# whatshap/whatshap

Hardware: AMD Instinct MI355X
Metric: variant-columns/sec at max-coverage 20 (bipartition-costs/sec reported alongside) (higher is better)
Workload: dtype u32; 1 GPU; synthetic diploid single-individual, max-coverage 20: 1 block of 200000 SNVs (BASELINE configs[2]); blocks=1, blocks_in_flight_per_gpu=1, tables_per_launch=1, max_coverage=20, optimal_cost_checksum=1611545, rendezvous=none

## Files before the change

### whatshap_amd/csrc/dp_device.hip

```cpp
#include <hip/hip_runtime.h>

#include <algorithm>
#include <atomic>
#include <cctype>
#include <chrono>
#include <cstdio>
#include <cstdlib>
#include <cstring>
#include <mutex>
#include <string>
#include <vector>

#include "debug_build.h"
#include "device_pool.h"
#include "device_table.h"
#include "genotype.h"

namespace whamd {

#define HIP_TRY(expr)                                                                                 \
	do {                                                                                              \
		hipError_t err_ = (expr);                                                                     \
		if (err_ != hipSuccess) {                                                                     \
			msg = std::string(#expr) + " failed: " + hipGetErrorString(err_);                         \
// ... 516 lines not shown
		schedule.clear();
		entries.clear();
		slot_entries.clear();
		windows.clear();
	}

	void release() {
		if (tail_elsewhere && ev3) (void)hipEventSynchronize(ev3);
		tail_elsewhere = false;
		if (upload_pending && ev_upload) (void)hipEventSynchronize(ev_upload);
		upload_pending = false;
		release_lanes();
		windowed = false;
		if (stream && own_stream_used && (!allocations.empty() || d_arena)) { (void)hipStreamSynchronize(stream); own_stream_used = false; }
		for (auto& a : allocations) devpool_give(device, a.first, a.second);
		allocations.clear();
		arena_give(device, d_arena, arena_bytes);
		d_arena = nullptr;
		arena_bytes = 0;
		pinned_give(h_pinned, h_pinned_bytes);
		h_pinned = nullptr;
		d_cols = nullptr;
		d_units = nullptr;
		d_pr[0] = d_pr[1] = nullptr;
		d_path_index = d_path_trans = d_score = nullptr;
	}
};

DeviceTable::DeviceTable() : impl_(new Impl()) {}

DeviceTable::~DeviceTable() {
	if (impl_) {
		release_device();
		delete impl_;
	}
}

void DeviceTable::release_device() {
	Impl& m = *impl_;
	(void)hipSetDevice(m.device);
	m.release();
	if (m.stream) {
		if (m.own_stream_used) (void)hipStreamSynchronize(m.stream);
		m.own_stream_used = false;
		StreamSet ss;
		ss.stream = m.stream; ss.ev[0] = m.ev0; ss.ev[1] = m.ev1; ss.ev[2] = m.ev2; ss.ev[3] = m.ev3; ss.ev[4] = m.ev_group; ss.ev[5] = m.ev_upload; ss.device = m.device;
		streamset_give(ss);
	}
	m.stream = m.run_stream = nullptr;
	m.ev0 = m.ev1 = m.ev2 = m.ev3 = m.ev_group = m.ev_upload = nullptr;
	m.timing_pending = false;
}

int DeviceTable::device_count() {
	int n = 0;
	if (hipGetDeviceCount(&n) != hipSuccess) return 0;
	return n;
}

bool DeviceTable::device_pci_bus_id(int device, std::string& out) {
	int n = 0;
	if (hipGetDeviceCount(&n) != hipSuccess || device < 0 || device >= n) return false;
	char text[64] = {0};
	if (hipDeviceGetPCIBusId(text, (int)sizeof text - 1, device) != hipSuccess) return false;
	out = text;
	for (char& ch : out) ch = (char)tolower((unsigned char)ch);
	return true;
}

static void append_segments(uint32_t mask, std::vector<uint32_t>& out, uint16_t& count) {
	uint32_t src = 0;
	count = 0;
	for (uint32_t bit = 0; bit < 32;) {
		if (!((mask >> bit) & 1u)) { ++bit; continue; }
		uint32_t len = 0;
		while (bit + len < 32 && ((mask >> (bit + len)) & 1u)) ++len;
		out.push_back(src | (bit << 8) | (len << 16));
		++count;
		src += len;
		bit += len;
	}
}

bool DeviceTable::set_path(const std::string& path) {
	if (path != "auto" && path != "column" && path != "column_keys" && path != "resident" && path != "slots") return false;
	impl_->path = path;
	return true;
}

void DeviceTable::set_l_pref(int l) { impl_->l_pref = std::max(4, std::min(l, RES_LMAX)); }
void DeviceTable::set_lanes(int n) { impl_->max_lanes = n < 1 ? 1 : (n > 64 ? 64 : n); }

void DeviceTable::set_fold(bool v) { impl_->fold = v; }
void DeviceTable::set_slot_l(int l) { impl_->slot_l = std::max(2, std::min(l, 12)); impl_->slot_l_set = true; }
void DeviceTable::set_slot_lr(int lr) { impl_->slot_lr = lr >= 3 ? 3 : (lr <= 1 ? 1 : 2); }

void DeviceTable::set_arena_limit(uint64_t bytes) { impl_->arena_limit = bytes; }
void DeviceTable::set_shared_launches(bool v) { impl_->shared_hint = v; }
void DeviceTable::set_side_by_side(bool v) { impl_->side_by_side = v; }
void DeviceTable::set_symmetry(int level) { impl_->symmetry = level < 0 ? 0 : (level > 2 ? 2 : level); }

whamd_status_t DeviceTable::upload(Problem& p, int device, std::string& msg) {
	Impl& m = *impl_;
	m.device = device;
	int ndev = 0;
	if (hipGetDeviceCount(&ndev) != hipSuccess || ndev <= 0) {
		msg = "no HIP device visible: the whatshap_amd device path needs an MI355X (gfx950); there is no CPU fallback";
		return WHAMD_ERR_DEVICE;
	}
	if (device < 0 || device >= ndev) {
		msg = "device index " + std::to_string(device) + " out of range (" + std::to_string(ndev) + " visible)";
		return WHAMD_ERR_DEVICE;
	}
	HIP_TRY(hipSetDevice(device));
	if (!m.stream) {
		StreamSet ss;
		if (!streamset_take(device, ss)) { msg = "could not create the table's stream and events"; return WHAMD_ERR_DEVICE; }
		m.stream = ss.stream; m.ev0 = ss.ev[0]; m.ev1 = ss.ev[1]; m.ev2 = ss.ev[2]; m.ev3 = ss.ev[3]; m.ev_group = ss.ev[4]; m.ev_upload = ss.ev[5];
	}
	m.release();
	const uint32_t n = p.n_cols;
	if (n == 0) return WHAMD_OK;
	m.wide = !select_kernels(p.T, p.n_ind, m.fused, m.keysfn);
	if (m.wide && (p.T > (uint32_t)MAX_T_WIDE || p.n_ind > (uint32_t)MAX_IND_WIDE)) {
		msg = "no device kernel for T=" + std::to_string(p.T) + ", individuals=" + std::to_string(p.n_ind);
		return WHAMD_ERR_UNSUPPORTED;
	}
	for (uint32_t c = 0; c < p.n_cols && !m.wide; ++c) m.wide = p.term_end(c, p.T - 1) - p.term_begin(c, 0) > (uint64_t)COL_MAXTERMS;
	const bool force_keys = m.path == "column_keys" || m.wide;
	const bool want_resident = (m.path == "auto" || m.path == "resident") && !m.wide;
	const auto tu0 = std::chrono::steady_clock::now();
	size_t free_b = 0, total_b = 0;
	HIP_TRY(hipMemGetInfo(&free_b, &total_b));
	if (free_b < total_b / 2) {
		genotype_release_cache();
		HIP_TRY(hipMemGetInfo(&free_b, &total_b));
	}
	if (free_b < total_b / 4) {
		dptable_release_arena_cache();
		devpool_release();
		HIP_TRY(hipMemGetInfo(&free_b, &total_b));
	}
	free_b += arena_idle_bytes(device);
	int slot_lr = m.slot_lr, slot_l = m.slot_l;
	if (m.shared_hint && p.T == 1 && p.max_k >= 18 && !m.slot_l_set && m.slot_lr == 2) { slot_lr = 3; slot_l = 12; }
	if (p.T == 1 && p.max_k >= 21 && p.max_k <= 22 && !m.slot_l_set && m.slot_lr == 2 && !debug_env("WHAMD_NO_WIDE_LAYOUT")) { slot_lr = 3; slot_l = 12; }
	m.slot_lr_used = slot_lr;
	m.use_slots = (m.path == "auto" || m.path == "slots") && !m.wide && plan_forward_slots(p, p.T > 1 ? (m.slot_l_set ? -m.slot_l : 0) : std::max(8, slot_l), m.symmetry, m.splan, slot_lr);
	if (m.use_slots && m.splan.ped && m.splan.table_words * 4ull > free_b / 4) m.use_slots = false;
	m.table_bytes = m.use_slots && m.splan.ped ? m.splan.table_words * 4ull : 0ull;
	if (p.lazy_terms) {
		std::vector<uint8_t> need(p.n_cols, 1);
		if (m.use_slots && m.splan.ped) for (uint32_t c = 0; c < p.n_cols; ++c) need[c] = m.splan.col_to_row[c] < 0;
		const whamd_status_t st = fill_lazy_terms(p, need, msg);
		if (st != WHAMD_OK) return st;
	}
	if (m.use_slots) {
		m.plan = ResidentPlan();
		m.plan.steps = m.splan.steps;
		m.plan.component_first_step = m.splan.component_first_step;
		m.plan.col_to_res.assign(p.n_cols, -1);
	} else {
		m.splan = SlotPlan();
		plan_forward(p, want_resident, m.l_pref, m.fold, m.plan, m.symmetry);
	}
	const auto tu1 = std::chrono::steady_clock::now();
	if (debug_env("WHAMD_DEBUG_PLAN")) {
		for (const Step& st : m.plan.steps) {
			if (st.kind == 0) { fprintf(stderr, "[plan] column %u k=%u b=%u f=%u\n", st.index, p.k[st.index], p.b[st.index], p.f[st.index]); continue; }
			if (st.kind == 2) {
				const SlotRun& r = m.splan.runs[st.index];
				fprintf(stderr, "[plan] slot run c0=%u ncols=%u g=%u L=%u half=%u ends=%u has_prev=%u in_identity=%u in_half=%u mirror_pos=%u in_occ=%x out_occ=%x mirror_out=%u\n",
				        r.c0, r.ncols, r.g, r.L, r.half, r.n_ends, r.has_prev, r.in_identity, r.in_half, r.in_mirror_pos, r.in_occ, r.out_occ, r.mirror_out);
				if (m.splan.ped) fprintf(stderr, "[plan]   pedigree run: T=%u forms per value=%u table words=%u record words per workgroup=%u\n", 1u << m.splan.pextra[st.index].tb,
				                         m.splan.pextra[st.index].nf, m.splan.pextra[st.index].s_off + r.ncols * 64u * pslot_ns(m.splan.pextra[st.index].nf), m.splan.pextra[st.index].rec_words);
				continue;
			}
			const ResSegment& sgm = m.plan.segments[st.index];
			fprintf(stderr, "[plan] run c0=%u ncols=%u g=%u threads=%u max_l=%u stage_words=%u\n", sgm.c0, sgm.ncols, sgm.g, sgm.threads, sgm.max_l, sgm.stage_words);
			for (uint32_t i = 0; i < sgm.ncols; ++i) {
				const ResColumn& rc = m.plan.columns[sgm.col_off + i];
				const ResBacktrace& rb = m.plan.backtrace[sgm.col_off + i];
				fprintf(stderr, "[plan]   col %u mode=%u nfold=%u Lb=%u Lf=%u ebits=%u epos0=%u nthr=%u stage_off=%u nwords=%u | bt layout=%u n_g=%u n_l=%u\n",
				        sgm.c0 + i, rc.mode, rc.nfold, rc.Lb, rc.Lf, rc.ebits, rc.epos[0], rc.nthr, rc.stage_off, rc.nwords, rb.layout, rb.n_g, rb.n_l);
			}
		}
	}
	const uint32_t tbits = 2 * p.n_triples;
	const uint32_t ni = std::max<uint32_t>(p.n_ind, 1);
	const bool timing = getenv("WHAMD_DEBUG_TIMING") != nullptr;
	auto lap_t = std::chrono::steady_clock::now();
	auto ulap = [&](const char* what) {
		if (!timing) return;
		const auto now = std::chrono::steady_clock::now();
		fprintf(stderr, "[whamd timing]   upload: %s %.2f ms\n", what, std::chrono::duration<double, std::milli>(now - lap_t).count());
		lap_t = now;
	};
	m.cols.resize(n);
	std::vector<uint32_t> segs;
	RawVec<uint32_t> term_ptr32((size_t)n * (p.T + 1));
	static_assert(sizeof(CostTerm) == sizeof(DevTerm), "Problem::terms / fterms are uploaded as they are");
	const RawVec<CostTerm>& terms = p.terms;
	if (p.terms.size() >= 0xFFFFFFFFull || (uint64_t)p.col_ptr[n] * ni >= 0xFFFFFFFFull) {
		msg = "problem too large for 32-bit device offsets";
		return WHAMD_ERR_UNSUPPORTED;
	}
	uint64_t bt = 0, seg_bt = 0;
	size_t seg_cursor = 0, slot_cursor = 0;
	uint32_t max_f = 0, max_keys_f = 0;
	const uint64_t reserve = (3ull << 30) + (uint64_t)n * 1024ull + m.table_bytes;
	const bool ped_slots = m.use_slots && m.splan.ped;
	auto slot_record_bytes = [&](size_t ri) -> uint64_t {
		const SlotRun& run = m.splan.runs[ri];
		if (ped_slots) return (uint64_t)m.splan.pextra[ri].rec_words * 4ull << run.g;
		return (uint64_t)run.n_ends * run.threads * (1ull << (run.g - run.half));
	};
	uint64_t arena_cap = free_b > reserve ? free_b - reserve : 0;
	if (m.arena_limit) arena_cap = std::min<uint64_t>(arena_cap, m.arena_limit);
	std::vector<uint32_t> window_first_col;
	uint64_t bt_max = 0;
	auto open_unit = [&](uint32_t c, uint64_t bytes) -> bool {
		if (bytes + 16 > arena_cap) return false;
		if (bt + bytes + 16 > arena_cap) {
			bt_max = std::max(bt_max, bt);
			bt = 0;
			window_first_col.push_back(c);
		}
		return true;
	};
	auto unit_too_large = [&](uint32_t c) {
		msg = "the backtrace record of the unit at column " + std::to_string(c) + " alone does not fit in the arena (" + std::to_string(arena_cap >> 20) +
		      " MiB of " + std::to_string(free_b >> 20) + " MiB free HBM)";
		return WHAMD_ERR_UNSUPPORTED;
	};
	parallel_ranges(n, host_threads(n, 16384), [&](uint64_t c0, uint64_t c1, uint32_t) {
		for (uint32_t c = (uint32_t)c0; c < (uint32_t)c1; ++c) {
			DevColumn d{};
			d.k = p.k[c];
			d.b = p.b[c];
			d.f = p.f[c];
			d.recomb = p.recomb[c];
			d.delta_off = (uint32_t)(p.col_ptr[c] * ni);
			d.term_off = (uint32_t)((size_t)c * (p.T + 1));
			for (uint32_t t = 0; t <= p.T; ++t) term_ptr32[(size_t)c * (p.T + 1) + t] = (uint32_t)p.term_ptr[(size_t)c * p.T + t];
			d.ebits = d.k - d.f;
			d.is_last = (c + 1 == n);
			d.eloop = std::min<uint32_t>(d.ebits, QMAX);
			d.nplanes = d.ebits + tbits;
			m.cols[c] = d;
		}
	});
	for (uint32_t c = 0; c < n; ++c) {
		DevColumn& d = m.cols[c];
		const bool in_slot_run = m.use_slots && m.splan.col_to_row[c] >= 0;
		d.seg_off = (uint32_t)segs.size();
		const uint32_t kmask = d.k >= 32 ? 0xFFFFFFFFu : ((1u << d.k) - 1u);
		if (!in_slot_run) {
			append_segments(p.fwd_mask[c], segs, d.nseg_fwd);
			append_segments(kmask & ~p.fwd_mask[c], segs, d.nseg_end);
		}
		d.bt_off = bt;
		if (m.use_slots && m.splan.col_to_row[c] >= 0) {
			d.mode = 3;
			d.res_idx = (uint32_t)m.splan.col_to_row[c];
			if (slot_cursor < m.splan.runs.size() && m.splan.runs[slot_cursor].c0 == c) {
				SlotRun& run = m.splan.runs[slot_cursor];
				if (!open_unit(c, slot_record_bytes(slot_cursor))) return unit_too_large(c);
				run.rec_lo = (uint32_t)bt;
				run.rec_hi = (uint32_t)(bt >> 32);
				seg_bt = bt;
				bt += slot_record_bytes(slot_cursor);
				max_f = std::max(max_f, run.L + run.g);
				++slot_cursor;
			}
			d.bt_off = seg_bt;
		} else if (m.plan.col_to_res[c] >= 0) {
			d.mode = 2;
			d.res_idx = (uint32_t)m.plan.col_to_res[c];
			if (seg_cursor < m.plan.segments.size() && m.plan.segments[seg_cursor].c0 == c) {
				ResSegment& sgm = m.plan.segments[seg_cursor];
				if (!open_unit(c, (uint64_t)sgm.stage_words * (1ull << sgm.g) * 8ull)) return unit_too_large(c);
				sgm.bt_lo = (uint32_t)bt;
				sgm.bt_hi = (uint32_t)(bt >> 32);
				seg_bt = bt;
				bt += (uint64_t)sgm.stage_words * (1ull << sgm.g) * 8ull;
				++seg_cursor;
			}
			d.bt_off = seg_bt;
		} else {
			const bool fused_ok = !force_keys && !d.is_last && d.f >= 6 && d.ebits <= (uint32_t)QMAX;
			d.mode = fused_ok ? 0u : 1u;
			const uint64_t bytes = d.mode == 0 ? (uint64_t)d.nplanes * p.T * (1ull << (d.f - 6)) * 8ull : (uint64_t)p.T * (1ull << d.f) * 4ull;
			if (!open_unit(c, bytes)) return unit_too_large(c);
			d.bt_off = bt;
			bt += bytes;
			if (d.mode != 0) max_keys_f = std::max(max_keys_f, d.f);
		}
		bt = (bt + 15ull) & ~15ull;
		max_f = std::max(max_f, d.f);
	}
	ulap("column descriptors (host)");
	bt = bt_max = std::max(bt_max, bt);
	m.bt_bytes = bt;
	m.windowed = !window_first_col.empty();
	m.checkpoint_bytes = (size_t)(1ull << max_f) * p.T * 4;
	const uint64_t need = bt + (2ull + window_first_col.size()) * (1ull << max_f) * p.T * 4ull + (1ull << max_keys_f) * p.T * 8ull;
	if (need + (1ull << 30) > free_b) {
		msg = "backtrace arena of " + std::to_string(need >> 20) + " MiB does not fit in free HBM (" + std::to_string(free_b >> 20) + " MiB)";
		return WHAMD_ERR_UNSUPPORTED;
	}
	hipStream_t us = debug_env("WHAMD_UPLOAD_ON_TABLE_STREAM") ? nullptr : upload_stream_of(device);
	if (!us) us = m.stream;
	m.upload_stream = us;
	if (us == m.stream) m.own_stream_used = true;
	StageSession stage(us);
	ulap("staging area taken");
	auto alloc = [&](void** dptr, size_t bytes) -> hipError_t {
		size_t got = 0;
		hipError_t e = devpool_take(device, std::max<size_t>(bytes, 16), dptr, &got);
		if (e == hipSuccess) m.allocations.emplace_back(*dptr, got);
		return e;
	};
	std::vector<int32_t> delta_fallback;
	const int32_t* delta_src = p.delta.data();
	size_t delta_count = (size_t)p.col_ptr[n] * p.n_ind;
	if (p.n_ind == 0) { delta_fallback.assign(std::max<size_t>(p.col_ptr[n], 1), 0); delta_src = delta_fallback.data(); delta_count = delta_fallback.size(); }
	void *d_delta, *d_term_ptr, *d_terms, *d_segs, *d_bt, *d_keys, *d_last_keys, *d_rcol, *d_rbt, *d_fterms = nullptr;
	m.device_superreads = n > 0 && p.n_ind == 1 && p.T == 1 && p.P == 2 && !p.distrust && p.h2p.size() >= 2 && p.h2p[0] == 0 && p.h2p[1] == 1 && p.genotype.size() >= n &&
	                      !debug_env("WHAMD_HOST_SUPERREADS");
	const size_t super_upload = m.device_superreads ? ((size_t)n + 1) * 8 + n + 1024 : 0;
	const size_t upload_bytes = m.cols.size() * sizeof(DevColumn) + delta_count * sizeof(int32_t) + term_ptr32.size() * 4 + (terms.size() + p.fterms.size()) * sizeof(DevTerm) + segs.size() * 4 +
	             m.plan.columns.size() * (sizeof(ResColumn) + sizeof(ResBacktrace) + sizeof(PedColumn)) + m.plan.ped_terms.size() * sizeof(PedTerm) +
	             (m.splan.rows.size() + SLOT_ROW_PAD) * sizeof(SlotRow) + m.splan.prows.size() * sizeof(PedSlotRow) + m.splan.bt_cols.size() * (sizeof(SlotBtCol) + 8) +
	             m.splan.runs.size() * (sizeof(SlotRun) + sizeof(PedSlotExtra) + sizeof(BtUnit) + sizeof(SlotBatchEntry) + 64) + m.plan.segments.size() * (sizeof(ResBatchEntry) + sizeof(BtUnit)) + super_upload + ((size_t)8 << 20);
	stage.expect(upload_bytes);
// ... 103 lines not shown
		m.super_words = (size_t)n + ((size_t)2 * n + 3) / 4;
	}
	if (!p.fterms.empty()) HIP_TRY(up(&d_fterms, p.fterms.data(), p.fterms.size() * sizeof(DevTerm)));
	HIP_TRY(up(&d_segs, segs.data(), segs.size() * sizeof(uint32_t)));
	HIP_TRY(up(&d_rcol, m.plan.columns.data(), m.plan.columns.size() * sizeof(ResColumn)));
	HIP_TRY(up(&d_rbt, m.plan.backtrace.data(), m.plan.backtrace.size() * sizeof(ResBacktrace)));
	void *d_pcol = nullptr, *d_pterm = nullptr;
	m.plan.ped_columns.resize(m.plan.ped_columns.empty() ? 0 : m.plan.columns.size());
	HIP_TRY(up(&d_pcol, m.plan.ped_columns.data(), m.plan.ped_columns.size() * sizeof(PedColumn)));
	HIP_TRY(up(&d_pterm, m.plan.ped_terms.data(), m.plan.ped_terms.size() * sizeof(PedTerm)));
	m.dp.ped_cols = (const PedColumn*)d_pcol;
	m.dp.ped_terms = (const PedTerm*)d_pterm;
	ulap("column arrays: allocations + copies");
	RawVec<uint32_t> slot_blob;
	std::vector<uint32_t> slot_blob_off(m.splan.runs.size(), 0), slot_blob_words(m.splan.runs.size(), 0);
	{
		size_t words = 0;
		for (size_t ri = 0; ri < m.splan.runs.size(); ++ri) {
			const SlotRun& run = m.splan.runs[ri];
			slot_blob_off[ri] = (uint32_t)words;
			slot_blob_words[ri] = (uint32_t)((size_t)run.ncols * (sizeof(SlotBtCol) / 4) + (run.n_ends + 3) / 4 + 1);
			words += slot_blob_words[ri];
		}
		slot_blob.resize(words);
		parallel_ranges(m.splan.runs.size(), host_threads(m.splan.runs.size(), 512), [&](uint64_t r0, uint64_t r1, uint32_t) {
			for (size_t ri = r0; ri < r1; ++ri) {
				const SlotRun& run = m.splan.runs[ri];
				uint32_t* dst = slot_blob.data() + slot_blob_off[ri];
				const size_t col_words = (size_t)run.ncols * (sizeof(SlotBtCol) / 4);
				std::memcpy(dst, m.splan.bt_cols.data() + run.row_off, col_words * 4);
				const size_t end_words = (run.n_ends + 3) / 4 + 1;
				std::memset(dst + col_words, 0, end_words * 4);
				if (run.n_ends) std::memcpy(dst + col_words, m.splan.end_slots.data() + m.splan.end_off[ri], run.n_ends);
			}
		});
	}
	ulap("slot backtrace blobs (host)");
	void *d_srows = nullptr, *d_sblob = nullptr;
	if (!m.splan.rows.empty()) m.splan.rows.resize(m.splan.rows.size() + SLOT_ROW_PAD);
	HIP_TRY(up(&d_srows, m.splan.rows.data(), m.splan.rows.size() * sizeof(SlotRow)));
	ulap("slot rows: allocation + copy");
	HIP_TRY(up(&d_sblob, slot_blob.data(), slot_blob.size() * sizeof(uint32_t)));
	void* d_sctrl = nullptr;
	HIP_TRY(up(&d_sctrl, m.splan.ctrl.data(), m.splan.ctrl.size() * sizeof(uint32_t)));
	m.dp.slot_ctrl = (const uint32_t*)d_sctrl;
	void *d_sruns = nullptr, *d_stab = nullptr;
	uint64_t slot_tab_words = 0;
	if (m.use_slots && !ped_slots) {
		for (SlotRun& run : m.splan.runs) {
			auto pad4 = [](uint64_t v) { return (v + 3ull) & ~3ull; };
			const bool xrun = (run.yflags & 1u) && (run.lr == 2u || (run.lr == 3u && !debug_env("WHAMD_NO_XRUN8"))) && run.ncols <= (uint32_t)SLOT_XCOLS &&
			                  run.n_ends <= (uint32_t)SLOT_XENDS && !debug_env("WHAMD_NO_XRUN");
			const uint64_t ncp = xrun ? ((run.ncols + 7u) & ~7u) : run.ncols;
			run.tab_g = (uint32_t)slot_tab_words;
			slot_tab_words += pad4(ncp << (run.g - run.half));
			run.tab_w = (uint32_t)slot_tab_words;
			slot_tab_words += pad4(ncp * (run.threads >> 6));
			run.tab_sl = (uint32_t)slot_tab_words;
			slot_tab_words += ncp * 64u;
			if (xrun) {
				run.yflags |= 8u;
				slot_tab_words = (slot_tab_words + 15u) & ~(uint64_t)15;
				run.tab_kr = (uint32_t)slot_tab_words;
				slot_tab_words += pad4((((uint64_t)run.ncols + SLOT_XPAD) << run.lr) + run.ncols + SLOT_XPAD);
				run.tab_par = (uint32_t)slot_tab_words;
				slot_tab_words += pad4((uint64_t)run.threads + (1ull << (run.g - run.half)));
			}
		}
		slot_tab_words += (uint64_t)SLOT_XCOLS * 64u;
		if (getenv("WHAMD_DEBUG_TIMING")) {
			size_t nx = 0, not_y = 0, not_lr = 0, long_run = 0, many_ends = 0;
			for (const SlotRun& run : m.splan.runs) {
				nx += (run.yflags & 8u) != 0;
				not_y += !(run.yflags & 1u); not_lr += run.lr != 2u && run.lr != 3u; long_run += run.ncols > (uint32_t)SLOT_XCOLS; many_ends += run.n_ends > (uint32_t)SLOT_XENDS;
			}
			fprintf(stderr, "[whamd timing]   X runs: %zu of %zu (not Y form %zu, cells per thread %zu, more than %d columns %zu, more than %d ending reads %zu)\n", nx, m.splan.runs.size(), not_y,
			        not_lr, SLOT_XCOLS, long_run, SLOT_XENDS, many_ends);
		}
		if (slot_tab_words >= 0xFFFFFFFFull) { msg = "slot-run tables exceed 32-bit offsets"; return WHAMD_ERR_UNSUPPORTED; }
		HIP_TRY(up(&d_sruns, m.splan.runs.data(), m.splan.runs.size() * sizeof(SlotRun)));
		ulap("slot blobs, control words, runs: allocations + copies");
		HIP_TRY(alloc(&d_stab, slot_tab_words * 4));
		ulap("slot tables: allocation");
	}
	m.dp.slot_tab = (const uint32_t*)d_stab;
	void *d_prows = nullptr, *d_pruns = nullptr, *d_pextra = nullptr, *d_ptab = nullptr;
	if (ped_slots) {
		HIP_TRY(up(&d_prows, m.splan.prows.data(), m.splan.prows.size() * sizeof(PedSlotRow)));
		HIP_TRY(up(&d_pruns, m.splan.runs.data(), m.splan.runs.size() * sizeof(SlotRun)));
		HIP_TRY(up(&d_pextra, m.splan.pextra.data(), m.splan.pextra.size() * sizeof(PedSlotExtra)));
		HIP_TRY(alloc(&d_ptab, m.table_bytes));
	}
	m.dp.pslot_rows = (const PedSlotRow*)d_prows;
	m.dp.pslot_tab = (const uint32_t*)d_ptab;
	m.dp.slot_rows = (const SlotRow*)d_srows;
	m.dp.slot_blob = (const uint32_t*)d_sblob;
	ulap("slot rows / blobs / control words: allocations + copies");
	m.release_lanes();
	{
		Impl::Job final_job;
		final_job.final = true;
		std::vector<Impl::Job> component_jobs;
		const std::vector<uint32_t>& first = m.plan.component_first_step;
		size_t largest = 0;
		for (size_t k = 0; k < first.size(); ++k) largest = std::max<size_t>(largest, (k + 1 < first.size() ? first[k + 1] : m.plan.steps.size()) - first[k]);
		const bool worth_splitting = largest * 5 < m.plan.steps.size() * 4 || debug_env("WHAMD_SPLIT_COMPONENTS");
		const bool split = m.max_lanes > 1 && first.size() > 1 && worth_splitting && !debug_env("WHAMD_DEBUG_STAMPS") && !m.windowed;
		if (!split) {
			for (uint32_t si = 0; si < m.plan.steps.size(); ++si) final_job.steps.push_back(si);
		} else {
			for (size_t k = 0; k < first.size(); ++k) {
				const uint32_t s0 = first[k], s1 = k + 1 < first.size() ? first[k + 1] : (uint32_t)m.plan.steps.size();
				Impl::Job* job = &final_job;
				if (k + 1 < first.size()) { component_jobs.emplace_back(); job = &component_jobs.back(); }
				for (uint32_t si = s0; si < s1; ++si) job->steps.push_back(si);
			}
		}
		m.jobs.push_back(std::move(final_job));
		for (Impl::Job& j : component_jobs) m.jobs.push_back(std::move(j));
	}
	{
		m.units.clear();
		for (Impl::Job& job : m.jobs) {
		job.unit_off = (uint32_t)m.units.size();
		for (size_t sj = job.steps.size(); sj-- > 0;) {
			const Step& st = m.plan.steps[job.steps[sj]];
			BtUnit u{};
			u.kind = st.kind;
			if (st.kind == 0) {
				const DevColumn& d = m.cols[st.index];
				u.c0 = st.index;
				u.ncols = 1;
				u.g = d.f; u.Lf_last = d.mode; u.stage_words = d.nplanes; u.n_wext = d.ebits;
				u.bt_lo = (uint32_t)d.bt_off; u.bt_hi = (uint32_t)(d.bt_off >> 32);
				u.n_lext = d.nseg_fwd; u.pad0 = d.nseg_end;
				const uint32_t nseg = (uint32_t)d.nseg_fwd + d.nseg_end;
				if (nseg <= (uint32_t)(RES_IOSEG + RES_BT_LRUNS)) {
					uint32_t* dst = u.wext;
					for (uint32_t i = 0; i < nseg; ++i) dst[i] = segs[d.seg_off + i];
					u.pad1[0] = 1;
				}
			} else if (st.kind == 2) {
				const SlotRun& run = m.splan.runs[st.index];
				SlotBtUnit su{};
				su.kind = ped_slots ? 3 : 2; su.c0 = run.c0; su.ncols = run.ncols; su.blob_off = slot_blob_off[st.index];
				su.g = run.g; su.L = run.L; su.n_ends = run.n_ends; su.threads = run.threads;
				su.bt_lo = run.rec_lo; su.bt_hi = run.rec_hi; su.half = run.half; su.blob_words = slot_blob_words[st.index];
				su.f_exit = m.splan.f_exit[st.index];
				for (uint32_t j = 0; j < su.f_exit && j < 32; ++j) su.exit_pos[j] = (uint8_t)slot_pos(run.out_pos, m.splan.exit_slot[st.index][j]);
				su.lr = run.lr;
				if (ped_slots) { su.n_ends = m.splan.pextra[st.index].rec_words; su.lr = m.splan.pextra[st.index].tb; }
				for (uint32_t j = 0; j < su.f_exit && j < 32; ++j) su.exit_slot[j] = m.splan.exit_slot[st.index][j];
				static_assert(sizeof(SlotBtUnit) == sizeof(BtUnit), "unit headers share one array");
				std::memcpy(&u, &su, sizeof u);
			} else {
				const ResSegment& sgm = m.plan.segments[st.index];
				u.c0 = sgm.c0; u.ncols = sgm.ncols; u.col_off = sgm.col_off; u.g = sgm.g; u.Lf_last = sgm.Lf_last;
				u.stage_words = sgm.stage_words; u.n_wext = sgm.n_wext; u.bt_lo = sgm.bt_lo; u.bt_hi = sgm.bt_hi;
				u.n_lext = sgm.n_lext;
				u.pad0 = (uint32_t)sgm.bt_active | ((uint32_t)sgm.bt_simple << 16) | (sgm.half << 20);
				std::copy(sgm.wext, sgm.wext + RES_IOSEG, u.wext);
				std::copy(sgm.lext, sgm.lext + RES_BT_LRUNS, u.lext);
			}
			m.units.push_back(u);
		}
		job.unit_count = (uint32_t)m.units.size() - job.unit_off;
		}
	}
	if (m.windowed) {
		const std::vector<uint32_t>& steps = m.jobs[0].steps;
		const uint32_t n_steps = (uint32_t)steps.size();
		auto first_col = [&](uint32_t pos) {
			const Step& st = m.plan.steps[steps[pos]];
			return st.kind == 0 ? st.index : (st.kind == 2 ? m.splan.runs[st.index].c0 : m.plan.segments[st.index].c0);
		};
		Impl::Window w;
		size_t next = 0;
		for (uint32_t pos = 0; pos < n_steps; ++pos) {
			if (next < window_first_col.size() && first_col(pos) == window_first_col[next]) {
				w.step_hi = pos;
				m.windows.push_back(w);
				w = Impl::Window();
				w.step_lo = pos;
				++next;
			}
		}
		w.step_hi = n_steps;
		m.windows.push_back(w);
		if (next != window_first_col.size()) { msg = "internal error: a window does not start at a step"; return WHAMD_ERR_DEVICE; }
		std::vector<BtJob> wjobs;
		for (size_t wi = 0; wi < m.windows.size(); ++wi) {
			Impl::Window& win = m.windows[wi];
			win.unit_off = n_steps - win.step_hi;
			win.unit_count = win.step_hi - win.step_lo;
			wjobs.push_back(BtJob{win.unit_off, win.unit_count, wi + 1 == m.windows.size() ? 1u : 2u, 0u});
		}
		void* d_wjobs = nullptr;
		HIP_TRY(up(&d_wjobs, wjobs.data(), wjobs.size() * sizeof(BtJob)));
		m.d_window_jobs = (BtJob*)d_wjobs;
		HIP_TRY(alloc((void**)&m.d_checkpoints, (m.windows.size() - 1) * m.checkpoint_bytes));
		HIP_TRY(alloc((void**)&m.d_bt_state, 16));
		if (getenv("WHAMD_DEBUG_TIMING")) fprintf(stderr, "[whamd timing] windowed solve: %zu windows, arena %.2f GB\n", m.windows.size(), (double)bt / 1e9);
	}
	m.super_off = 2 * (size_t)n + 4 + m.jobs.size();
	{
		void* d_res = nullptr;
		HIP_TRY(alloc(&d_res, (m.super_off + (m.device_superreads ? m.super_words : 0)) * sizeof(uint32_t) + 16));
		uint32_t* res = (uint32_t*)d_res;
		m.d_path_index = res;
		m.d_path_trans = res + n;
		m.d_score = res + 2 * (size_t)n;
		m.d_job_scores = res + 2 * (size_t)n;
		m.d_bt_counters = res + 2 * (size_t)n + m.jobs.size();
		if (m.device_superreads) {
			m.super_args.out = res + m.super_off;
			m.super_args.path_index = m.d_path_index;
		}
	}
	m.use_chunks = false;
	m.chunks.clear();
	m.n_spec = 0;
	for (SlotRun& run : m.splan.runs) run.spec_id = 0;
	const bool trio_runs = !m.use_slots && !m.plan.ped_columns.empty();
	if (trio_runs) for (ResSegment& sgm : m.plan.segments) sgm.in_mirror_bit = 0;
	if ((m.use_slots || trio_runs) && m.jobs.size() == 1 && !m.windowed && !getenv("WHAMD_BT_SEQUENTIAL") && m.units.size() > 2u * BT_CHUNK_RUNS) {
		m.use_chunks = true;
		std::vector<int> generator_of(std::max<uint32_t>(p.n_ind, 1), -1);
		std::vector<uint32_t> generator_tflip;
		if (p.n_ind >= 2 && p.n_ind <= BT_GENERATORS) {
			for (uint32_t s = 0; s < p.n_ind; ++s) {
				uint32_t as_parent = 0, as_child = 0;
				for (uint32_t t3 = 0; t3 < p.n_triples; ++t3) {
					if (p.triples[t3][0] == s) as_parent |= 1u << (2 * t3);
					if (p.triples[t3][1] == s) as_parent |= 1u << (2 * t3 + 1);
					if (p.triples[t3][2] == s) as_child |= 3u << (2 * t3);
				}
				if (as_parent && as_child) continue;
				if (!as_parent && !as_child) continue;
				generator_of[s] = (int)generator_tflip.size();
				generator_tflip.push_back(as_parent | as_child);
			}
		}
		auto orientations = [&](BtChunk& ch, uint32_t unit) {
			const BtUnit& bu = m.units[unit];
			const uint32_t c_last = bu.c0 + bu.ncols - 1;
			ch.n_orient = 1;
			for (uint32_t q = 0; q < BT_GENERATORS; ++q) ch.flip[q] = 0;
			if (p.n_triples == 0 && p.n_ind <= 1) {
				const uint32_t fb = p.f[c_last];
// ... 167 lines not shown
						: ((size_t)e.sg.ncols * (64 + RES_TABLE) * 4 + 2 * ((size_t)4 << e.sg.max_l) + (size_t)e.sg.stage_words * 8);
					ss.lds = std::max(ss.lds, lds);
					ss.grid_x = std::max(ss.grid_x, 1u << (e.sg.g - e.sg.half));
					ss.threads = std::max(ss.threads, e.sg.threads);
					ss.sym = ss.sym || e.sg.half || e.sg.in_half || e.sg.mirror_out;
					m.entries.push_back(e);
					++ss.entry_count;
				} else {
					ss.singles.push_back(Impl::Single{(uint32_t)li, si, c.flip, first, (last && !job.final) ? (int32_t)job_id : -1});
					ss.io[0] = lane.d_pr[c.flip]; ss.io[1] = lane.d_pr[c.flip ^ 1];
				}
				c.flip ^= 1;
				if (last) { ++c.job_i; c.step_i = 0; } else ++c.step_i;
			}
			if (!ss.entry_count && ss.singles.empty()) break;
			m.max_grid_x = std::max(m.max_grid_x, ss.grid_x * std::max(1u, ss.entry_count));
			m.schedule.push_back(std::move(ss));
		}
		if (m.windowed) {
			if (m.schedule.size() != m.jobs[0].steps.size()) { msg = "internal error: windowed schedule"; return WHAMD_ERR_DEVICE; }
			const size_t nw = m.windows.size();
			for (size_t wi = 0; wi + 1 < nw; ++wi) m.schedule[m.windows[wi].step_hi - 1].ck_save = (int32_t)wi;
			m.schedule.back().bt_window = (int32_t)(nw - 1);
			for (size_t wi = nw - 1; wi-- > 0;) {
				const Impl::Window& win = m.windows[wi];
				for (uint32_t pos = win.step_lo; pos < win.step_hi; ++pos) {
					Impl::SuperStep again = m.schedule[pos];
					again.ck_save = -1;
					again.ck_load = (pos == win.step_lo && wi > 0) ? (int32_t)(wi - 1) : -1;
					again.bt_window = pos + 1 == win.step_hi ? (int32_t)wi : -1;
					m.schedule.push_back(std::move(again));
				}
			}
		}
		m.step_brief.clear();
		m.entry_brief.clear();
		if (m.use_slots) {
			m.step_brief.reserve(m.schedule.size());
			m.entry_brief.reserve(m.slot_entries.size());
			for (const Impl::SuperStep& ss : m.schedule) {
				m.step_brief.push_back(Impl::StepBrief{(uint32_t)m.entry_brief.size(), (uint32_t)ss.lds, (uint16_t)ss.entry_count, (uint8_t)(ss.singles.empty() ? 0 : 1), 0});
				for (uint32_t q = 0; q < ss.entry_count; ++q) {
					const SlotBatchEntry& he = m.slot_entries[ss.entry_off + q];
					Impl::EntryBrief eb{};
					eb.grid_x = (uint16_t)(1u << (he.run.g - he.run.half));
					eb.threads = (uint16_t)he.run.threads;
					eb.lds_x = (uint32_t)((size_t)2 * he.run.threads * (4u << he.run.lr));
					if (m.splan.ped) eb.variant = eb.variant_x = (uint8_t)(he.ex.nf == (uint32_t)PSLOT_FACT4 ? 10 : he.ex.nf == (uint32_t)PSLOT_FACT ? 7 : (he.ex.nf == 16 ? 5 : 1 + (he.ex.tb == 4 ? 2 : 0) + (he.ex.nf == 4 ? 1 : 0)));
					else {
						eb.variant = (uint8_t)(he.run.lr == 3 ? 6 : 0);
						eb.variant_x = (he.run.yflags & 8u) ? (uint8_t)(he.run.lr == 3 ? 9 : 8) : eb.variant;
					}
					m.entry_brief.push_back(eb);
				}
			}
		}
		void* d_entries = nullptr;
		HIP_TRY(up(&d_entries, m.entries.data(), m.entries.size() * sizeof(ResBatchEntry)));
		m.d_entries = (ResBatchEntry*)d_entries;
		void* d_slot_entries = nullptr;
		m.slot_entries.resize(m.slot_entries.size() + 2);
		HIP_TRY(up(&d_slot_entries, m.slot_entries.data(), m.slot_entries.size() * sizeof(SlotBatchEntry)));
		m.slot_entries.resize(m.slot_entries.size() - 2);
		m.d_slot_entries = (SlotBatchEntry*)d_slot_entries;
		std::vector<BtJob> btjobs;
		for (const Impl::Job& job : m.jobs) btjobs.push_back(BtJob{job.unit_off, job.unit_count, job.final ? 1u : 0u, 0u});
		void* d_btjobs = nullptr;
		HIP_TRY(up(&d_btjobs, btjobs.data(), btjobs.size() * sizeof(BtJob)));
		m.d_btjobs = (BtJob*)d_btjobs;
	}
	HIP_TRY(flush_slab());
	m.dp.cols = m.d_cols;
	m.dp.term_ptr = (const uint32_t*)d_term_ptr;
	m.dp.terms = (const DevTerm*)d_terms;
	if (ped_slots) {
		uint32_t most = 0;
		for (size_t ri = 0; ri < m.splan.runs.size(); ++ri)
			most = std::max<uint32_t>(most, (m.splan.pextra[ri].fwn << m.splan.runs[ri].g) + (m.splan.pextra[ri].fwn << m.splan.runs[ri].lw) + m.splan.runs[ri].ncols * (64u * pslot_ns(m.splan.pextra[ri].nf) + p.T * pslot_nk(m.splan.pextra[ri].nf)));
		const uint32_t bx = std::max(1u, std::min(1024u, (most + 255u) / 256u));
		for (size_t r0 = 0; r0 < m.splan.runs.size(); r0 += 32768) {
			const uint32_t ny = (uint32_t)std::min<size_t>(32768, m.splan.runs.size() - r0);
			hipLaunchKernelGGL(pedslot_tables, dim3(bx, ny), dim3(256), 0, us, m.dp, (const SlotRun*)d_pruns + r0, (const PedSlotExtra*)d_pextra + r0, (uint32_t*)d_ptab,
			                   (const DevTerm*)d_fterms);
		}
		HIP_TRY(hipGetLastError());
	}
	if (m.use_slots && !ped_slots && !m.splan.runs.empty()) {
		uint32_t most = 0;
		for (const SlotRun& run : m.splan.runs) most = std::max<uint32_t>(most, ((run.ncols + 8u) << (run.g - run.half)) + (run.ncols + 8u) * ((run.threads >> 6) + 64u));
		const uint32_t bx = std::max(1u, std::min(64u, (most + 255u) / 256u));
		for (size_t r0 = 0; r0 < m.splan.runs.size(); r0 += 32768) {
			const uint32_t ny = (uint32_t)std::min<size_t>(32768, m.splan.runs.size() - r0);
			hipLaunchKernelGGL(slot_tables, dim3(bx, ny), dim3(256), 0, us, m.dp, (const SlotRun*)d_sruns + r0, (uint32_t*)d_stab);
		}
		HIP_TRY(hipGetLastError());
	}
	HIP_TRY(hipEventRecord(m.ev_upload, us));
	m.upload_pending = true;
	if (debug_env("WHAMD_SYNC_UPLOAD") || unstaged_copies || !stage.image || !stage.park()) {
		HIP_TRY(hipStreamSynchronize(us));
		stage.finish();
	}
	m.dp.delta = (const int32_t*)d_delta;
	m.dp.term_ptr = (const uint32_t*)d_term_ptr;
	m.dp.terms = (const DevTerm*)d_terms;
	m.dp.segs = (const uint32_t*)d_segs;
	m.dp.bt = (uint8_t*)d_bt;
	m.dp.keys = (unsigned long long*)d_keys;
	m.dp.last_keys = (unsigned long long*)d_last_keys;
	m.dp.bt_state = m.windowed ? m.d_bt_state : nullptr;
	m.dp.res_cols = (const ResColumn*)d_rcol;
	m.dp.res_bt = (const ResBacktrace*)d_rbt;
	m.dp.dbg = nullptr;
	if (getenv("WHAMD_DEBUG_TIMING")) {
		auto ms = [](std::chrono::steady_clock::time_point a, std::chrono::steady_clock::time_point b) { return std::chrono::duration<double, std::milli>(b - a).count(); };
		fprintf(stderr, "[whamd timing] upload: plan %.1f ms, descriptors + copies %.1f ms, backtrace arena (%.2f GB) %.1f ms, rest %.1f ms\n",
		        ms(tu0, tu1), ms(tu1, tu2), (double)bt / 1e9, ms(tu2, tu3), ms(tu3, std::chrono::steady_clock::now()));
	}
	if (debug_env("WHAMD_DEBUG_STAMPS") && !m.use_slots) {
		void* d_dbg = nullptr;
		const size_t dbg_bytes = (m.plan.segments.size() + 1) * 64 + 4 * 512 * 16 + 64;
		HIP_TRY(alloc(&d_dbg, dbg_bytes));
		HIP_TRY(hipMemset(d_dbg, 0, dbg_bytes));
		m.dp.dbg = (unsigned long long*)d_dbg;
		m.dp.dbg_wg_off = (uint32_t)((m.plan.segments.size() + 1) * 8);
		m.dp.dbg_flags = (uint32_t)atoi(debug_env("WHAMD_DEBUG_STAMPS"));
	}
	if (debug_env("WHAMD_SLOT_STAMPS") && m.use_slots) {
		void* d_dbg = nullptr;
		const size_t dbg_bytes = (m.splan.runs.size() + 1) * 48 * 8 + 4 * 512 * 16 + 128;
		HIP_TRY(alloc(&d_dbg, dbg_bytes));
		HIP_TRY(hipMemset(d_dbg, 0, dbg_bytes));
		m.dp.dbg = (unsigned long long*)d_dbg;
		m.dp.dbg_wg_off = (uint32_t)((m.splan.runs.size() + 1) * 48);
		for (size_t i = 0; i < m.slot_entries.size(); ++i) m.slot_entries[i].run.pad = (uint32_t)i;
	}
	if (const char* skip = debug_env("WHAMD_SLOT_SKIP")) m.dp.dbg_flags = (uint32_t)atoi(skip);
	m.dp.n_cols = n;
	m.dp.T = p.T;
	m.dp.tbits = tbits;
	m.dp.n_ind = p.n_ind;
	{
		static std::mutex attr_mu;
		static unsigned long long attr_done = 0;
		std::lock_guard<std::mutex> lock(attr_mu);
		if (device >= 64 || !((attr_done >> device) & 1ull)) {
		HIP_TRY(hipFuncSetAttribute(reinterpret_cast<const void*>(resident_segment<false, false>), hipFuncAttributeMaxDynamicSharedMemorySize, 160 * 1024));
		HIP_TRY(hipFuncSetAttribute(reinterpret_cast<const void*>(resident_segment<false, true>), hipFuncAttributeMaxDynamicSharedMemorySize, 160 * 1024));
#ifdef WHAMD_DEBUG_BUILD
		HIP_TRY(hipFuncSetAttribute(reinterpret_cast<const void*>(resident_segment<true, true>), hipFuncAttributeMaxDynamicSharedMemorySize, 160 * 1024));
#endif
		HIP_TRY(hipFuncSetAttribute(reinterpret_cast<const void*>(resident_batch<false>), hipFuncAttributeMaxDynamicSharedMemorySize, 160 * 1024));
		HIP_TRY(hipFuncSetAttribute(reinterpret_cast<const void*>(resident_batch<true>), hipFuncAttributeMaxDynamicSharedMemorySize, 160 * 1024));
		HIP_TRY(hipFuncSetAttribute(reinterpret_cast<const void*>(backtrace_kernel), hipFuncAttributeMaxDynamicSharedMemorySize, 160 * 1024));
		HIP_TRY(hipFuncSetAttribute(reinterpret_cast<const void*>(resident_segment_ped<false>), hipFuncAttributeMaxDynamicSharedMemorySize, 160 * 1024));
#ifdef WHAMD_DEBUG_BUILD
		HIP_TRY(hipFuncSetAttribute(reinterpret_cast<const void*>(resident_segment_ped<true>), hipFuncAttributeMaxDynamicSharedMemorySize, 160 * 1024));
#endif
		HIP_TRY(hipFuncSetAttribute(reinterpret_cast<const void*>((resident_segment_ped<false, true>)), hipFuncAttributeMaxDynamicSharedMemorySize, 160 * 1024));
		HIP_TRY(hipFuncSetAttribute(reinterpret_cast<const void*>((slot_runx<2, 24, false, false>)), hipFuncAttributeMaxDynamicSharedMemorySize, 160 * 1024));
		HIP_TRY(hipFuncSetAttribute(reinterpret_cast<const void*>((slot_runx<2, 24, false, true>)), hipFuncAttributeMaxDynamicSharedMemorySize, 160 * 1024));
		HIP_TRY(hipFuncSetAttribute(reinterpret_cast<const void*>((slot_runx<2, 32, false, false>)), hipFuncAttributeMaxDynamicSharedMemorySize, 160 * 1024));
		HIP_TRY(hipFuncSetAttribute(reinterpret_cast<const void*>((slot_runx<2, 32, false, true>)), hipFuncAttributeMaxDynamicSharedMemorySize, 160 * 1024));
		HIP_TRY(hipFuncSetAttribute(reinterpret_cast<const void*>((slot_runx<2, 0, false, false>)), hipFuncAttributeMaxDynamicSharedMemorySize, 160 * 1024));
		HIP_TRY(hipFuncSetAttribute(reinterpret_cast<const void*>((slot_runx<2, 0, false, true>)), hipFuncAttributeMaxDynamicSharedMemorySize, 160 * 1024));
		HIP_TRY(hipFuncSetAttribute(reinterpret_cast<const void*>((slot_runx<2, 8, false, false>)), hipFuncAttributeMaxDynamicSharedMemorySize, 160 * 1024));
		HIP_TRY(hipFuncSetAttribute(reinterpret_cast<const void*>((slot_runx<2, 8, false, true>)), hipFuncAttributeMaxDynamicSharedMemorySize, 160 * 1024));
		HIP_TRY(hipFuncSetAttribute(reinterpret_cast<const void*>((slot_runx<2, 16, false, false>)), hipFuncAttributeMaxDynamicSharedMemorySize, 160 * 1024));
		HIP_TRY(hipFuncSetAttribute(reinterpret_cast<const void*>((slot_runx<2, 16, false, true>)), hipFuncAttributeMaxDynamicSharedMemorySize, 160 * 1024));
		HIP_TRY(hipFuncSetAttribute(reinterpret_cast<const void*>((slot_groupx<2, false>)), hipFuncAttributeMaxDynamicSharedMemorySize, 160 * 1024));
		HIP_TRY(hipFuncSetAttribute(reinterpret_cast<const void*>((slot_groupx<3, false>)), hipFuncAttributeMaxDynamicSharedMemorySize, 160 * 1024));
#ifdef WHAMD_DEBUG_BUILD
		HIP_TRY(hipFuncSetAttribute(reinterpret_cast<const void*>((slot_runx<2, 24, true, false>)), hipFuncAttributeMaxDynamicSharedMemorySize, 160 * 1024));
		HIP_TRY(hipFuncSetAttribute(reinterpret_cast<const void*>((slot_runx<2, 24, true, true>)), hipFuncAttributeMaxDynamicSharedMemorySize, 160 * 1024));
		HIP_TRY(hipFuncSetAttribute(reinterpret_cast<const void*>((slot_runx<2, 32, true, false>)), hipFuncAttributeMaxDynamicSharedMemorySize, 160 * 1024));
		HIP_TRY(hipFuncSetAttribute(reinterpret_cast<const void*>((slot_runx<2, 32, true, true>)), hipFuncAttributeMaxDynamicSharedMemorySize, 160 * 1024));
// ... 712 lines not shown
```

Measured before the change: 2.240 million variant-columns/s.

## Parallelize host column descriptor, segment and backtrace layout construction

Result: slower. 2.215 million variant-columns/s (median of 2 runs) (-1.1%).

```diff
diff --git a/whatshap_amd/csrc/dp_device.hip b/whatshap_amd/csrc/dp_device.hip
--- a/whatshap_amd/csrc/dp_device.hip
+++ b/whatshap_amd/csrc/dp_device.hip
@@ -622,6 +622,19 @@
 	}
 }
 
+static void write_segments(uint32_t mask, uint32_t* out, uint16_t& count) {
+	uint32_t src = 0;
+	count = 0;
+	for (uint32_t bit = 0; bit < 32;) {
+		if (!((mask >> bit) & 1u)) { ++bit; continue; }
+		uint32_t len = 0;
+		while (bit + len < 32 && ((mask >> (bit + len)) & 1u)) ++len;
+		out[count++] = src | (bit << 8) | (len << 16);
+		src += len;
+		bit += len;
+	}
+}
+
 bool DeviceTable::set_path(const std::string& path) {
 	if (path != "auto" && path != "column" && path != "column_keys" && path != "resident" && path != "slots") return false;
 	impl_->path = path;
@@ -773,7 +786,22 @@
 		      " MiB of " + std::to_string(free_b >> 20) + " MiB free HBM)";
 		return WHAMD_ERR_UNSUPPORTED;
 	};
-	parallel_ranges(n, host_threads(n, 16384), [&](uint64_t c0, uint64_t c1, uint32_t) {
+	const uint32_t n_desc = host_threads(n, 16384);
+	std::vector<int32_t> unit_at;
+	if (m.use_slots) {
+		unit_at.assign(n, -1);
+		for (size_t ri = 0; ri < m.splan.runs.size(); ++ri) if (m.splan.runs[ri].c0 < n) unit_at[m.splan.runs[ri].c0] = (int32_t)ri;
+	} else if (!m.plan.segments.empty()) {
+		unit_at.assign(n, -1);
+		for (size_t si = 0; si < m.plan.segments.size(); ++si) if (m.plan.segments[si].c0 < n) unit_at[m.plan.segments[si].c0] = (int32_t)si;
+	}
+	auto starts_unit = [&](uint32_t c) { return !unit_at.empty() && unit_at[c] >= 0; };
+	auto count_segments = [](uint32_t mask) { return (uint16_t)__builtin_popcount(mask & ~(mask << 1)); };
+	RawVec<uint64_t> own_bt(n);
+	struct DescRange { uint64_t bt = 0, segs = 0, last_start = 0, units = 0; bool has_start = false; uint32_t max_f = 0, max_keys_f = 0; };
+	std::vector<DescRange> desc_range(n_desc);
+	parallel_ranges(n, n_desc, [&](uint64_t c0, uint64_t c1, uint32_t t) {
+		DescRange& dr = desc_range[t];
 		for (uint32_t c = (uint32_t)c0; c < (uint32_t)c1; ++c) {
 			DevColumn d{};
 			d.k = p.k[c];
@@ -787,10 +815,97 @@
 			d.is_last = (c + 1 == n);
 			d.eloop = std::min<uint32_t>(d.ebits, QMAX);
 			d.nplanes = d.ebits + tbits;
+			uint64_t own = 0;
+			if (!(m.use_slots && m.splan.col_to_row[c] >= 0)) {
+				const uint32_t kmask = d.k >= 32 ? 0xFFFFFFFFu : ((1u << d.k) - 1u);
+				d.nseg_fwd = count_segments(p.fwd_mask[c]);
+				d.nseg_end = count_segments(kmask & ~p.fwd_mask[c]);
+				dr.segs += (uint64_t)d.nseg_fwd + d.nseg_end;
+			}
+			if (m.use_slots && m.splan.col_to_row[c] >= 0) {
+				d.mode = 3;
+				d.res_idx = (uint32_t)m.splan.col_to_row[c];
+				if (starts_unit(c)) {
+					const SlotRun& run = m.splan.runs[unit_at[c]];
+					own = slot_record_bytes((size_t)unit_at[c]);
+					dr.max_f = std::max(dr.max_f, run.L + run.g);
+					dr.has_start = true;
+					dr.last_start = dr.bt;
+					++dr.units;
+				}
+			} else if (m.plan.col_to_res[c] >= 0) {
+				d.mode = 2;
+				d.res_idx = (uint32_t)m.plan.col_to_res[c];
+				if (starts_unit(c)) {
+					const ResSegment& sgm = m.plan.segments[unit_at[c]];
+					own = (uint64_t)sgm.stage_words * (1ull << sgm.g) * 8ull;
+					dr.has_start = true;
+					dr.last_start = dr.bt;
+					++dr.units;
+				}
+			} else {
+				const bool fused_ok = !force_keys && !d.is_last && d.f >= 6 && d.ebits <= (uint32_t)QMAX;
+				d.mode = fused_ok ? 0u : 1u;
+				own = d.mode == 0 ? (uint64_t)d.nplanes * p.T * (1ull << (d.f - 6)) * 8ull : (uint64_t)p.T * (1ull << d.f) * 4ull;
+				if (d.mode != 0) dr.max_keys_f = std::max(dr.max_keys_f, d.f);
+			}
+			own_bt[c] = (own + 15ull) & ~15ull;
+			dr.bt += own_bt[c];
+			dr.max_f = std::max(dr.max_f, d.f);
 			m.cols[c] = d;
 		}
 	});
-	for (uint32_t c = 0; c < n; ++c) {
+	std::vector<uint64_t> bt_base(n_desc + 1, 0), seg_base(n_desc + 1, 0), seg_bt_in(n_desc, 0);
+	uint64_t units_found = 0;
+	for (uint32_t t = 0; t < n_desc; ++t) {
+		bt_base[t + 1] = bt_base[t] + desc_range[t].bt;
+		seg_base[t + 1] = seg_base[t] + desc_range[t].segs;
+		if (t + 1 < n_desc) seg_bt_in[t + 1] = desc_range[t].has_start ? bt_base[t] + desc_range[t].last_start : seg_bt_in[t];
+		units_found += desc_range[t].units;
+		max_f = std::max(max_f, desc_range[t].max_f);
+		max_keys_f = std::max(max_keys_f, desc_range[t].max_keys_f);
+	}
+	const uint64_t units_planned = m.use_slots ? m.splan.runs.size() : m.plan.segments.size();
+	const bool one_piece = bt_base[n_desc] + 16 <= arena_cap && units_found == units_planned;
+	if (one_piece) {
+		segs.resize(seg_base[n_desc]);
+		parallel_ranges(n, n_desc, [&](uint64_t c0, uint64_t c1, uint32_t t) {
+			uint64_t at = bt_base[t], run_at = seg_bt_in[t];
+			uint32_t* seg_out = segs.data() + seg_base[t];
+			for (uint32_t c = (uint32_t)c0; c < (uint32_t)c1; ++c) {
+				DevColumn& d = m.cols[c];
+				d.seg_off = (uint32_t)(seg_out - segs.data());
+				if (!(m.use_slots && m.splan.col_to_row[c] >= 0)) {
+					const uint32_t kmask = d.k >= 32 ? 0xFFFFFFFFu : ((1u << d.k) - 1u);
+					uint32_t one[32];
+					uint16_t cnt = 0;
+					write_segments(p.fwd_mask[c], one, cnt);
+					seg_out = std::copy(one, one + cnt, seg_out);
+					write_segments(kmask & ~p.fwd_mask[c], one, cnt);
+					seg_out = std::copy(one, one + cnt, seg_out);
+				}
+				d.bt_off = at;
+				if (d.mode >= 2 && starts_unit(c)) {
+					if (d.mode == 3) {
+						SlotRun& run = m.splan.runs[unit_at[c]];
+						run.rec_lo = (uint32_t)at;
+						run.rec_hi = (uint32_t)(at >> 32);
+					} else {
+						ResSegment& sgm = m.plan.segments[unit_at[c]];
+						sgm.bt_lo = (uint32_t)at;
+						sgm.bt_hi = (uint32_t)(at >> 32);
+					}
+					run_at = at;
+				}
+				if (d.mode >= 2) d.bt_off = run_at;
+				at += own_bt[c];
+			}
+		});
+		bt = bt_base[n_desc];
+	} else {
+		max_f = max_keys_f = 0;
+	}
+	for (uint32_t c = 0; c < n && !one_piece; ++c) {
 		DevColumn& d = m.cols[c];
 		const bool in_slot_run = m.use_slots && m.splan.col_to_row[c] >= 0;
 		d.seg_off = (uint32_t)segs.size();
@@ -1060,6 +1175,19 @@
 		ulap("slot blobs, control words, runs: allocations + copies");
 		HIP_TRY(alloc(&d_stab, slot_tab_words * 4));
 		ulap("slot tables: allocation");
+		if (!m.splan.runs.empty()) {
+			HIP_TRY(flush_slab());
+			uint32_t most = 0;
+			for (const SlotRun& run : m.splan.runs) most = std::max<uint32_t>(most, ((run.ncols + 8u) << (run.g - run.half)) + (run.ncols + 8u) * ((run.threads >> 6) + 64u));
+			const uint32_t bx = std::max(1u, std::min(64u, (most + 255u) / 256u));
+			DevProblem tp = m.dp;
+			tp.slot_rows = (const SlotRow*)d_srows;
+			for (size_t r0 = 0; r0 < m.splan.runs.size(); r0 += 32768) {
+				const uint32_t ny = (uint32_t)std::min<size_t>(32768, m.splan.runs.size() - r0);
+				hipLaunchKernelGGL(slot_tables, dim3(bx, ny), dim3(256), 0, us, tp, (const SlotRun*)d_sruns + r0, (uint32_t*)d_stab);
+			}
+			HIP_TRY(hipGetLastError());
+		}
 	}
 	m.dp.slot_tab = (const uint32_t*)d_stab;
 	void *d_prows = nullptr, *d_pruns = nullptr, *d_pextra = nullptr, *d_ptab = nullptr;
@@ -1098,11 +1226,14 @@
 		for (Impl::Job& j : component_jobs) m.jobs.push_back(std::move(j));
 	}
 	{
-		m.units.clear();
+		size_t n_units = 0;
 		for (Impl::Job& job : m.jobs) {
-		job.unit_off = (uint32_t)m.units.size();
-		for (size_t sj = job.steps.size(); sj-- > 0;) {
-			const Step& st = m.plan.steps[job.steps[sj]];
+			job.unit_off = (uint32_t)n_units;
+			job.unit_count = (uint32_t)job.steps.size();
+			n_units += job.steps.size();
+		}
+		m.units.assign(n_units, BtUnit{});
+		auto make_unit = [&](const Step& st) -> BtUnit {
 			BtUnit u{};
 			u.kind = st.kind;
 			if (st.kind == 0) {
@@ -1140,9 +1271,13 @@
 				std::copy(sgm.wext, sgm.wext + RES_IOSEG, u.wext);
 				std::copy(sgm.lext, sgm.lext + RES_BT_LRUNS, u.lext);
 			}
-			m.units.push_back(u);
-		}
-		job.unit_count = (uint32_t)m.units.size() - job.unit_off;
+			return u;
+		};
+		for (const Impl::Job& job : m.jobs) {
+			const size_t count = job.steps.size();
+			parallel_ranges(count, host_threads(count, 1024), [&](uint64_t i0, uint64_t i1, uint32_t) {
+				for (size_t i = i0; i < i1; ++i) m.units[job.unit_off + i] = make_unit(m.plan.steps[job.steps[count - 1 - i]]);
+			});
 		}
 	}
 	if (m.windowed) {
@@ -1476,16 +1611,6 @@
 			const uint32_t ny = (uint32_t)std::min<size_t>(32768, m.splan.runs.size() - r0);
 			hipLaunchKernelGGL(pedslot_tables, dim3(bx, ny), dim3(256), 0, us, m.dp, (const SlotRun*)d_pruns + r0, (const PedSlotExtra*)d_pextra + r0, (uint32_t*)d_ptab,
 			                   (const DevTerm*)d_fterms);
-		}
-		HIP_TRY(hipGetLastError());
-	}
-	if (m.use_slots && !ped_slots && !m.splan.runs.empty()) {
-		uint32_t most = 0;
-		for (const SlotRun& run : m.splan.runs) most = std::max<uint32_t>(most, ((run.ncols + 8u) << (run.g - run.half)) + (run.ncols + 8u) * ((run.threads >> 6) + 64u));
-		const uint32_t bx = std::max(1u, std::min(64u, (most + 255u) / 256u));
-		for (size_t r0 = 0; r0 < m.splan.runs.size(); r0 += 32768) {
-			const uint32_t ny = (uint32_t)std::min<size_t>(32768, m.splan.runs.size() - r0);
-			hipLaunchKernelGGL(slot_tables, dim3(bx, ny), dim3(256), 0, us, m.dp, (const SlotRun*)d_sruns + r0, (uint32_t*)d_stab);
 		}
 		HIP_TRY(hipGetLastError());
 	}
```
